# ivclab/CPG

Measured on AMD Instinct MI355X. Metric: images/sec per CPG train-prune-retrain cycle, VGG16 task-1, higher is better.
Workload: dtype f32; 1 GPU; configs[1]: VGG16-BN custom_vgg 224x224, task-1 CPG cycle (finetune -> prune 0.0->0.1 -> recovery, validate after every 20th train step), batch 256 per GPU; task=1, arch=vgg16, global_batch=256, per_gpu_batch=256, parallelism=dp1, epoch_steps=20

## Files before the change

cpg_amd/_lib.py:

```python
import ctypes
import os
import sys

import torch

_HERE = os.path.dirname(os.path.abspath(__file__))
LIB_PATH = os.environ.get('CPG_HIP_LIB') or os.path.join(_HERE, 'lib', 'libcpg_hip.so')

ABI_VERSION = 3
CPG_OK = 0
CPG_E_KRANGE = 2
CPG_E_INVALID = -1
MODE_FINETUNE = 0
MODE_PRUNE = 1



class ConvDesc(ctypes.Structure):
    _fields_ = [(n, ctypes.c_int32) for n in
                ('N', 'C', 'H', 'W', 'K', 'R', 'S', 'stride_h', 'stride_w', 'pad_h', 'pad_w', 'dil_h', 'dil_w', 'groups')]


class PruneResult(ctypes.Structure):
    _fields_ = [('n_candidates', ctypes.c_int64), ('k', ctypes.c_int64), ('n_released', ctypes.c_int64),
# ... 101 lines not shown
    'cpg_conv2d_dgrad_bf16x3': (_int, [_desc, _vp, _vp, _vp, _f32, _vp, _vp, _sz, _vp]),
    'cpg_conv2d_wgrad_bf16x3': (_int, [_desc, _vp, _vp, _vp, _vp, _f32, _vp, _vp, _vp, _sz, _vp]),
    'cpg_conv2d_dgrad_bf16': (_int, [_desc, _vp, _vp, _vp, _f32, _vp, _vp, _sz, _vp]),
    'cpg_conv2d_dgrad_bnbwd_tiles': (_i32, [_desc]),
    'cpg_conv2d_dgrad_bnbwd': (_int, [_desc, _vp, _vp, _vp, _f32, _vp, _vp, _vp, _vp, _vp, _vp, _vp, _sz, _vp, _sz, _vp]),
    'cpg_bn_bwd_from_partials': (_int, [_vp, _i32, _vp, _vp, _vp, _vp, _vp, _vp, _vp, _vp, _vp, _i32, _i32, _i32, _vp, _sz, _vp]),
    'cpg_bn_bwd_finalize_partials': (_int, [_vp, _i32, _i32, _i32, _i32, _vp, _vp, _vp, _vp]),
    'cpg_stem_bn_supported': (_i32, [_desc]),
    'cpg_stem_bn_tiles': (_i32, [_desc]),
    'cpg_stem_bn_stats': (_int, [_desc, _vp, _vp, _vp, _f32, _vp, _vp, _sz, _vp]),
    'cpg_stem_bn_relu_fwd': (_int, [_desc, _vp, _vp, _vp, _f32, _vp, _vp, _vp, _vp, _vp, _vp, _vp]),
    'cpg_stem_bn_relu_bwd_reduce': (_int, [_desc, _vp, _vp, _vp, _f32, _vp, _vp, _vp, _vp, _vp, _vp, _vp, _sz, _vp]),
    'cpg_stem_bn_relu_bwd_apply': (_int, [_desc, _vp, _vp, _vp, _f32, _vp, _vp, _vp, _vp, _vp, _vp, _vp, _vp, _vp]),
    'cpg_stem_bn_wgrad_workspace': (_sz, [_desc]),
    'cpg_stem_bn_relu_bwd_wgrad': (_int, [_desc, _vp, _vp, _vp, _f32, _vp, _vp, _vp, _vp, _vp, _vp, _vp, _vp, _vp, _vp, _sz, _vp]),
    'cpg_bn_stats_finalize_count': (_int, [_vp, _i32, _i32, _i32, _i32, _f32, _f32, _vp, _vp, _vp, _vp, _vp, _vp]),
    'cpg_bn_stats_finalize': (_int, [_vp, _i32, _i32, _i32, _i32, _f32, _f32, _vp, _vp, _vp, _vp, _vp]),
    'cpg_bn_add_relu_mask_bytes': (_sz, [_i32, _i32, _i32]),
    'cpg_bn_add_relu_fwd': (_int, [_vp, _vp, _vp, _vp, _f32, _f32, _vp, _vp, _vp, _vp, _vp, _i32, _i32, _i32, _i32, _vp, _sz, _vp, _vp]),
    'cpg_bn_relu_pool3_supported': (_i32, [_i32, _i32]),
    'cpg_bn_relu_pool3_fwd': (_int, [_vp] * 6 + [_i32] * 4 + [_vp]),
    'cpg_bn_relu_pool3_bwd': (_int, [_vp] * 9 + [_i32] * 5 + [_vp, _sz, _vp]),
    'cpg_bn_add_relu_bwd': (_int, [_vp] * 11 + [_i32] * 4 + [_vp, _sz, _vp, _vp]),
    'cpg_prelu_fwd': (_int, [_vp, _vp, _vp, _vp, _i32, _i32, _i32, _i32, _vp]),
    'cpg_prelu_bwd_bias': (_int, [_vp] * 6 + [_i32] * 4 + [_vp, _sz, _vp]),
    'cpg_prelu_workspace_bytes': (_sz, [_i32, _i32, _i32]),
    'cpg_prelu_bwd': (_int, [_vp, _vp, _vp, _vp, _vp, _i32, _i32, _i32, _i32, _vp, _sz, _vp]),
    'cpg_image_resample_workspace_bytes': (_sz, [ctypes.POINTER(ResampleItem), _i32]),
    'cpg_image_resample': (_int, [_vp, _i64, ctypes.POINTER(ResampleItem), _i32, _vp, _i64, _vp, _sz, _vp]),
    'cpg_image_to_tensor': (_int, [_vp, _i64, ctypes.POINTER(TensorItem), _i32, _i32, _i32, ctypes.POINTER(_f32), ctypes.POINTER(_f32), _vp,
# ... 126 lines not shown
```

cpg_amd/csrc/conv3x3_stem.hip:

```cpp
#include <algorithm>
#include <type_traits>
#include "cpg_dispatch.h"

using namespace cpg;

namespace {

typedef float f32x2 __attribute__((ext_vector_type(2)));
constexpr int ST_R = 8, ST_W = 32;
constexpr int ST_PW = 36;
constexpr int ST_ROWS = ST_R + 2;
constexpr int ST_CMAX = 3, ST_KS = 14;
constexpr int ST_PATCH = ST_CMAX * ST_ROWS * ST_PW;

struct StemGeom {
    int N, C, K, H, W;
    int tiles_x, tiles_y;
    unsigned ntiles;
};

enum { ST_PLAIN = 0, ST_STATS = 1, ST_STATS_ONLY = 2, ST_BN_RELU = 3, ST_BWD_REDUCE = 4, ST_BWD_APPLY = 5, ST_BWD_WGRAD = 6 };
constexpr int ST_TS = 36;
struct StemBn {
    const float *gamma, *beta, *mean, *invstd;
    const float *coef;
    const float *gz;
};

template <int MODE, int NB = 2, bool RAG = false>
__global__ __launch_bounds__(256, 2)
void k_stem_fwd(StemGeom g, const float *__restrict__ x, const float *__restrict__ w, const float *__restrict__ pm, float thr,
                const float *__restrict__ bias, float *__restrict__ y, float *__restrict__ stats, StemBn bn) {
    constexpr bool STATS = MODE == ST_STATS || MODE == ST_STATS_ONLY || MODE == ST_BWD_REDUCE;
    constexpr bool BN = MODE >= ST_BN_RELU;
    constexpr bool STORE = MODE == ST_PLAIN || MODE == ST_STATS || MODE == ST_BN_RELU || MODE == ST_BWD_APPLY;
    constexpr bool WG = MODE == ST_BWD_WGRAD;
    constexpr bool TWO_PASS = STATS || BN;
    __shared__ float smem_all[4 * ST_PATCH];
    __shared__ __attribute__((aligned(16))) float cst[(MODE >= ST_BWD_REDUCE) ? NB * 32 * 8 : 4];
    const int tid = threadIdx.x, lane = tid & 63, wave = __builtin_amdgcn_readfirstlane(tid >> 6);
    if constexpr (MODE >= ST_BWD_REDUCE) {
        if (tid < NB * 32) {
            const bool kv = tid < g.K;
            cst[tid * 8 + 0] = kv ? bn.mean[tid] : 0.0f, cst[tid * 8 + 1] = kv ? bn.invstd[tid] : 0.0f;
            cst[tid * 8 + 2] = kv ? bn.gamma[tid] : 0.0f, cst[tid * 8 + 3] = kv ? bn.beta[tid] : 0.0f;
            cst[tid * 8 + 4] = (MODE >= ST_BWD_APPLY && kv) ? bn.coef[2 * tid] : 0.0f;
            cst[tid * 8 + 5] = (MODE >= ST_BWD_APPLY && kv) ? bn.coef[2 * tid + 1] : 0.0f;
        }
        __syncthreads();
    }
    const int li = lane & 31, lh = lane >> 5;
    float *smem = smem_all + wave * ST_PATCH;
    const int HW = g.H * g.W, CK = g.C * 9;
    __shared__ __attribute__((aligned(16))) float tsm_all[WG ? 4 * 32 * ST_TS : 4];
    float *tsm = tsm_all + (WG ? wave * 32 * ST_TS : 0);
    const int wk = li < CK ? li : 0, wboff = ((wk / 9) * ST_ROWS + (wk % 9) / 3) * ST_PW + wk % 3 + lh;
    f32x16 accw[WG ? NB : 1];
    if constexpr (WG) {
#pragma unroll
        for (int mb = 0; mb < NB; ++mb)
#pragma unroll
            for (int e = 0; e < 16; ++e) accw[mb][e] = 0.0f;
    }

    constexpr bool ALDS = NB == 3 && TWO_PASS;
    __shared__ float a_lds[ALDS ? NB * ST_KS * 64 : 1];
    float A[ALDS ? 1 : NB][ST_KS];
    int boff[ST_KS];
#pragma unroll
    for (int t = 0; t < ST_KS; ++t) {
        const int k = 2 * t + lh;
        const bool kv = k < CK;
#pragma unroll
        for (int mb = 0; mb < NB; ++mb) {
            const int co = mb * 32 + li;
            float v = 0.0f;
            if (kv && co < g.K) {
                v = w[co * CK + k];
                if (pm != nullptr) v *= binarize(pm[co * CK + k], thr);
            }
// ... 46 lines not shown
            const int row = y0 - 1 + r, col = side ? x0 + ST_W : x0 - 1;
            const bool ok = item < ST_CMAX * ST_ROWS && c < g.C && (unsigned)row < (unsigned)g.H && (unsigned)col < (unsigned)g.W;
            const int off = ok ? (((n * g.C + c) * g.H + row) * g.W + col) * 4 : kOOR;
            ph = __builtin_bit_cast(float, __builtin_amdgcn_raw_buffer_load_b32(srd_x, off, 0, 0));
        }
    };
    auto write_patch = [&]() {
#pragma unroll
        for (int q = 0; q < 15; ++q) smem[(2 * q + hw_half) * ST_PW + 1 + hcol] = pc[q];
        if (lane < 2 * ST_CMAX * ST_ROWS) smem[(lane >> 1) * ST_PW + ((lane & 1) ? ST_W + 1 : 0)] = ph;
    };

    if constexpr (ALDS) __syncthreads();
    const unsigned nwaves = gridDim.x * 4, wid = blockIdx.x * 4 + wave;
    if (wid >= g.ntiles) return;
    const int HW4 = HW * 4;
    issue_loads(wid);
    for (unsigned tile = wid; tile < g.ntiles; tile += nwaves) {
        int n, y0, x0;
        tile_coords(tile, n, y0, x0);
        write_patch();
        if (tile + nwaves < g.ntiles) issue_loads(tile + nwaves);
        float s1[16], s2[16];
        auto zero_sums = [&]() {
            if (STATS) {
#pragma unroll
                for (int e = 0; e < 16; ++e) s1[e] = s2[e] = 0.0f;
            }
        };
        const __amdgpu_buffer_rsrc_t srd_y = __builtin_amdgcn_make_buffer_rsrc((void *)((STORE ? y : (float *)x) + (STORE ? (int64_t)n * g.K * HW : 0)), 0, STORE ? g.K * HW4 : 0, 0x00020000);
// ... 82 lines not shown
                    }
                    if constexpr (MODE == ST_STATS || MODE == ST_STATS_ONLY) {
                        const float vm = (FULL || pok) ? v : 0.0f;
                        s1[e] += vm;
                        s2[e] = fmaf(vm, vm, s2[e]);
                    }
                    if constexpr (MODE == ST_BN_RELU) {
                        const float z = relu_keep((v - cm[e]) * cis[e] * cga[e] + cbe[e]);
                        __builtin_amdgcn_raw_buffer_store_b32(__builtin_bit_cast(int, z), srd_y, voff_of(mb, e), cu * HW4, 0);
                    }
                    if constexpr (MODE >= ST_BWD_REDUCE) {
                        const float *cc = cst + (cu + 4 * lh) * 8 + copq;
                        const f32x4 c4 = *reinterpret_cast<const f32x4 *>(cc);
                        const float xh = (v - c4[0]) * c4[1];
                        const float gm = ((v - c4[0]) * c4[1] * c4[2] + c4[3] > 0.0f) ? gzv[e] : 0.0f;
                        if constexpr (MODE == ST_BWD_REDUCE) {
                            s1[e] += gm;
                            s2[e] = fmaf(gm, xh, s2[e]);
                        } else {
                            const f32x2 c2 = *reinterpret_cast<const f32x2 *>(cc + 4);
                            float gyv = (gm - c2[0] - xh * c2[1]) * (c4[1] * c4[2]);
                            if constexpr (MODE == ST_BWD_APPLY) {
                                __builtin_amdgcn_raw_buffer_store_b32(__builtin_bit_cast(int, gyv), srd_y, voff_of(mb, e), cu * HW4, 0);
                            } else {
                                if (!FULL && !pok) gyv = 0.0f;
                                tsm[((e & 3) + 8 * (e >> 2) + 4 * lh) * ST_TS + (li & 1) * 16 + (li >> 1)] = gyv;
                            }
                        }
                    }
                }
            if constexpr (WG) {
                f32x4 ga[4];
#pragma unroll
                for (int q = 0; q < 4; ++q) ga[q] = *reinterpret_cast<const f32x4 *>(tsm + li * ST_TS + lh * 16 + 4 * q);
                const float *brow = smem + j * ST_PW + wboff;
#pragma unroll
                for (int t = 0; t < 16; ++t)
                    accw[MB0] = __builtin_amdgcn_mfma_f32_32x32x2f32(ga[t >> 2][t & 3], brow[2 * t], accw[MB0], 0, 0, 0);
            }
        };
        auto rows = [&](auto mbsel) {
            if (full) {
#pragma unroll 1
                for (int j = 0; j < ST_R; ++j) row(j, std::true_type{}, mbsel);
            } else {
#pragma unroll 1
                for (int j = 0; j < ST_R; ++j) row(j, std::false_type{}, mbsel);
            }
        };
        auto stats_out = [&](int mb) {
#pragma unroll
            for (int e = 0; e < 16; e += 8) half_wave_sum8(s1 + e), half_wave_sum8(s2 + e);
            if (li == kHalfSumLane) {
#pragma unroll
                for (int e = 0; e < 16; ++e) {
                    const int co = mb * 32 + (e & 3) + 8 * (e >> 2) + 4 * lh;
                    if (RAG && co >= g.K) continue;
                    f32x2 o;
                    o[0] = s1[e], o[1] = s2[e];
                    *reinterpret_cast<f32x2 *>(stats + ((int64_t)co * g.ntiles + tile) * 2) = o;
                }
            }
        };
        if (TWO_PASS) {
            load_bn(0);
            zero_sums();
            rows(std::integral_constant<int, 0>{});
            if (STATS) stats_out(0);
            load_bn(1);
            zero_sums();
            rows(std::integral_constant<int, 1>{});
            if (STATS) stats_out(1);
            if constexpr (NB == 3) {
                load_bn(2);
                zero_sums();
                rows(std::integral_constant<int, 2>{});
                if (STATS) stats_out(2);
            }
        } else {
            rows(std::integral_constant<int, -1>{});
        }
    }
    if constexpr (WG) {
        float *dstw = y + (int64_t)wid * g.K * CK;
#pragma unroll
        for (int mb = 0; mb < NB; ++mb)
#pragma unroll
            for (int e = 0; e < 16; ++e) {
                const int co = mb * 32 + (e & 3) + 8 * (e >> 2) + 4 * lh;
                if (li < CK && co < g.K) dstw[co * CK + li] = accw[mb][e];
            }
    }
}

#define STEM_LAUNCH(MODE, grid, block, shm, stream, ...)                                                          \
    do {                                                                                                          \
        if (g.K == 64) hipLaunchKernelGGL((k_stem_fwd<MODE, 2, false>), grid, block, shm, stream, __VA_ARGS__);   \
        else hipLaunchKernelGGL((k_stem_fwd<MODE, 3, true>), grid, block, shm, stream, __VA_ARGS__);              \
    } while (0)

bool stem_geom(int N, int C, int K, int H, int W, StemGeom &g) {
    if (opt_on(OPT_NO_STEM)) return false;
    if (N < 1 || C < 1 || C > ST_CMAX || K < 64 || K > 96 || H < 1 || W < 1) return false;
    if ((int64_t)N * C * H * W * 4 >= (1ll << 31) || (int64_t)K * H * W * 4 >= (1ll << 31)) return false;
    g.N = N, g.C = C, g.K = K, g.H = H, g.W = W;
    g.tiles_x = (W + ST_W - 1) / ST_W, g.tiles_y = (H + ST_R - 1) / ST_R;
// ... 30 lines not shown
}

namespace {
bool stem_bn_geom(const cpg_conv_desc *d, StemGeom &g) {
    if (opt_on(OPT_NO_STEM_FUSE)) return false;
    if (!(d->R == 3 && d->S == 3 && d->stride_h == 1 && d->stride_w == 1 && d->pad_h == 1 && d->pad_w == 1 && d->dil_h == 1 &&
          d->dil_w == 1 && d->groups == 1))
        return false;
    return stem_geom(d->N, d->C, d->K, d->H, d->W, g);
}
unsigned stem_blocks(const StemGeom &g) {
    unsigned blocks = (unsigned)std::min<int64_t>(((int64_t)g.ntiles + 3) / 4, 4 * kCUs);
    blocks = (unsigned)std::max(1, opt_or(OPT_STEM_BLOCKS, (int)blocks));
    return blocks;
}
}

extern "C" int32_t cpg_stem_bn_supported(const cpg_conv_desc *d) {
    StemGeom g;
    return (d != nullptr && stem_bn_geom(d, g)) ? 1 : 0;
}
extern "C" int32_t cpg_stem_bn_tiles(const cpg_conv_desc *d) {
    StemGeom g;
    return (d != nullptr && stem_bn_geom(d, g)) ? (int32_t)g.ntiles : 0;
}
extern "C" int cpg_stem_bn_stats(const cpg_conv_desc *d, const float *x, const float *w, const float *pm, float thr, const float *bias,
                                 float *stats, size_t stats_bytes, void *stream_v) {
    StemGeom g;
    CPG_REQUIRE(d && x && w && stats, "cpg_stem_bn_stats: null pointer");
    if (!stem_bn_geom(d, g)) return fail(CPG_E_UNSUPPORTED, "cpg_stem_bn_stats: shape not supported");
// ... 7 lines not shown
extern "C" int cpg_stem_bn_relu_fwd(const cpg_conv_desc *d, const float *x, const float *w, const float *pm, float thr, const float *bias,
                                    const float *gamma, const float *beta, const float *mean, const float *invstd, float *z, void *stream_v) {
    StemGeom g;
    CPG_REQUIRE(d && x && w && gamma && beta && mean && invstd && z, "cpg_stem_bn_relu_fwd: null pointer");
    if (!stem_bn_geom(d, g)) return fail(CPG_E_UNSUPPORTED, "cpg_stem_bn_relu_fwd: shape not supported");
    if (bias != nullptr) return fail(CPG_E_UNSUPPORTED, "cpg_stem_bn_relu_fwd: the fused stem takes no conv bias");
    STEM_LAUNCH(ST_BN_RELU, dim3(stem_blocks(g)), dim3(256), 0, (hipStream_t)stream_v, g, x, w, pm, thr, bias, z,
                       (float *)nullptr, StemBn{gamma, beta, mean, invstd, nullptr, nullptr});
    CPG_CHECK_LAUNCH("cpg_stem_bn_relu_fwd");
    return CPG_OK;
}
extern "C" int cpg_stem_bn_relu_bwd_reduce(const cpg_conv_desc *d, const float *x, const float *w, const float *pm, float thr,
                                           const float *bias, const float *gamma, const float *beta, const float *mean, const float *invstd,
                                           const float *gz, float *partials, size_t partials_bytes, void *stream_v) {
    StemGeom g;
    CPG_REQUIRE(d && x && w && gamma && beta && mean && invstd && gz && partials, "cpg_stem_bn_relu_bwd_reduce: null pointer");
    if (!stem_bn_geom(d, g)) return fail(CPG_E_UNSUPPORTED, "cpg_stem_bn_relu_bwd_reduce: shape not supported");
    if (bias != nullptr) return fail(CPG_E_UNSUPPORTED, "cpg_stem_bn_relu_bwd_reduce: the fused stem takes no conv bias");
    if (partials_bytes < (size_t)g.K * g.ntiles * 2 * sizeof(float)) return fail(CPG_E_WORKSPACE, "cpg_stem_bn_relu_bwd_reduce: partial-sum buffer too small");
    STEM_LAUNCH(ST_BWD_REDUCE, dim3(stem_blocks(g)), dim3(256), 0, (hipStream_t)stream_v, g, x, w, pm, thr, bias,
                       (float *)nullptr, partials, StemBn{gamma, beta, mean, invstd, nullptr, gz});
    CPG_CHECK_LAUNCH("cpg_stem_bn_relu_bwd_reduce");
    return CPG_OK;
}
extern "C" int cpg_stem_bn_relu_bwd_apply(const cpg_conv_desc *d, const float *x, const float *w, const float *pm, float thr,
                                          const float *bias, const float *gamma, const float *beta, const float *mean, const float *invstd,
                                          const float *coef, const float *gz, float *gy, void *stream_v) {
    StemGeom g;
    CPG_REQUIRE(d && x && w && gamma && beta && mean && invstd && coef && gz && gy, "cpg_stem_bn_relu_bwd_apply: null pointer");
    if (!stem_bn_geom(d, g)) return fail(CPG_E_UNSUPPORTED, "cpg_stem_bn_relu_bwd_apply: shape not supported");
    if (bias != nullptr) return fail(CPG_E_UNSUPPORTED, "cpg_stem_bn_relu_bwd_apply: the fused stem takes no conv bias");
    STEM_LAUNCH(ST_BWD_APPLY, dim3(stem_blocks(g)), dim3(256), 0, (hipStream_t)stream_v, g, x, w, pm, thr, bias, gy,
                       (float *)nullptr, StemBn{gamma, beta, mean, invstd, coef, gz});
    CPG_CHECK_LAUNCH("cpg_stem_bn_relu_bwd_apply");
    return CPG_OK;
}

extern "C" size_t cpg_stem_bn_wgrad_workspace(const cpg_conv_desc *d) {
    StemGeom g;
    if (d == nullptr || !stem_bn_geom(d, g)) return 0;
    return (size_t)stem_blocks(g) * 4 * g.K * g.C * 9 * sizeof(float);
}
extern "C" int cpg_stem_bn_relu_bwd_wgrad(const cpg_conv_desc *d, const float *x, const float *w, const float *pm, float thr,
                                          const float *bias, const float *gamma, const float *beta, const float *mean, const float *invstd,
                                          const float *coef, const float *gz, float *gw, float *gpm, void *ws, size_t ws_bytes,
                                          void *stream_v) {
    StemGeom g;
    CPG_REQUIRE(d && x && w && gamma && beta && mean && invstd && coef && gz && gw && ws, "cpg_stem_bn_relu_bwd_wgrad: null pointer");
    CPG_REQUIRE((pm == nullptr) == (gpm == nullptr), "cpg_stem_bn_relu_bwd_wgrad: piggymask and its gradient come as a pair");
    if (!stem_bn_geom(d, g)) return fail(CPG_E_UNSUPPORTED, "cpg_stem_bn_relu_bwd_wgrad: shape not supported");
    if (bias != nullptr) return fail(CPG_E_UNSUPPORTED, "cpg_stem_bn_relu_bwd_wgrad: the fused stem takes no conv bias");
    const unsigned blocks = stem_blocks(g);
    if (ws_bytes < (size_t)blocks * 4 * g.K * g.C * 9 * sizeof(float)) return fail(CPG_E_WORKSPACE, "cpg_stem_bn_relu_bwd_wgrad: workspace too small");
    hipStream_t stream = (hipStream_t)stream_v;
    STEM_LAUNCH(ST_BWD_WGRAD, dim3(blocks), dim3(256), 0, stream, g, x, w, pm, thr, bias, (float *)ws, (float *)nullptr,
                       StemBn{gamma, beta, mean, invstd, coef, gz});
    const int nsplit = (int)std::min<int64_t>((int64_t)g.ntiles, (int64_t)blocks * 4);
    Epilogue ep{gw, nullptr, BIAS_NONE, 1, 1, pm, w, gpm, thr};
    launch_split_reduce((const float *)ws, nsplit, (int64_t)g.K * g.C * 9, 0, ep, stream);
    CPG_CHECK_LAUNCH("cpg_stem_bn_relu_bwd_wgrad");
    return CPG_OK;
}
```

cpg_amd/csrc/cpg_common.cpp:

```cpp
#include "cpg_common.h"
#include <stdarg.h>
#include <stdlib.h>
#include <string.h>
#include <atomic>

namespace cpg {

static thread_local char g_err[512] = "";

char *err_buf() { return g_err; }

int fail(int code, const char *fmt, ...) {
    va_list ap;
    va_start(ap, fmt);
    vsnprintf(g_err, sizeof(g_err), fmt, ap);
    va_end(ap);
    return code;
}

static thread_local PackCtx g_pack = {};
PackCtx &pack_ctx() { return g_pack; }
static thread_local WgradRider g_rider = {};
WgradRider &wgrad_rider() { return g_rider; }
static thread_local PoolMaxCtx g_pool_max = {};
PoolMaxCtx &pool_max_ctx() { return g_pool_max; }
static thread_local PoolMaxCtx g_bn_pool_max = {};
PoolMaxCtx &bn_pool_max_ctx() { return g_bn_pool_max; }

int take_packed(size_t bytes, const float **pre, const char *what) {
    PackCtx &c = g_pack;
    *pre = nullptr;
    if (!c.armed) return CPG_OK;
    if (c.use == nullptr || c.use_bytes != bytes || (((uintptr_t)c.use) & 15) != 0)
        return fail(CPG_E_INVALID, "%s: the packed operand handed in (%zu bytes) is not the one this launch streams (%zu bytes, 16-byte aligned)",
                    what, c.use_bytes, bytes);
    *pre = c.use;
    c.armed = false;
    return CPG_OK;
}

static std::atomic<int> g_shared_chip{0};
int shared_chip_hint() { return g_shared_chip.load(std::memory_order_relaxed); }
// ... 1 lines not shown
namespace {
enum Kind { BOOL, INT, WINO_KERNEL };
struct OptDef {
    const char *name;
    Kind kind;
};
const OptDef kDefs[OPT_COUNT] = {
    {"CPG_NO_WINO", BOOL},          {"CPG_NO_WINO_WGRAD", BOOL},   {"CPG_NO_WINO_ODD", BOOL},      {"CPG_NO_STEM", BOOL},
    {"CPG_NO_STEM_FUSE", BOOL},     {"CPG_NO_DEAD_SKIP", BOOL},    {"CPG_NO_S2", BOOL},            {"CPG_NO_V14", BOOL},
    {"CPG_DISABLE_CONV3X3", BOOL},  {"CPG_DISABLE_CONV1X1", BOOL}, {"CPG_DISABLE_CONV1X1_WGRAD", BOOL}, {"CPG_DISABLE_PW_GEMM", BOOL},
    {"CPG_C3_FORCE", INT},          {"CPG_C3W_BPC", INT},          {"CPG_W3_PICK", INT},           {"CPG_PWW_BPC", INT},
    {"CPG_STEM_BLOCKS", INT},       {"CPG_WINO_KERNEL", WINO_KERNEL}, {"CPG_WINO_NW", INT},        {"CPG_WINO_PERSIST", INT},
    {"CPG_WINO_GRIDS", INT},        {"CPG_WW_UNITS", INT},         {"CPG_WW_XCD", INT},            {"CPG_PW_TILE", INT},           {"CPG_WG3_SHARE", INT},
    {"CPG_WW_SHARE", INT},          {"CPG_WINO_TAIL", INT},         {"CPG_FC_SMALL", INT},
    {"CPG_NO_WW_RIDER", BOOL},      {"CPG_NO_GROUPED", BOOL},       {"CPG_GROUPED_WIDE_MIN", INT},
    {"CPG_NO_POOL_MAX", BOOL},
};

struct Table {
    std::atomic<int> v[OPT_COUNT];
    Table() {
        for (int i = 0; i < OPT_COUNT; ++i) {
            int val = OPT_UNSET;
            if (const char *f = getenv(kDefs[i].name)) {
                switch (kDefs[i].kind) {
                    case BOOL: val = (f[0] == 0 || (f[0] == '0' && f[1] == 0)) ? 0 : 1; break;
                    case INT: val = atoi(f); break;
                    case WINO_KERNEL: val = f[0] == 'b' ? 0 : f[0] == 'p' ? 2 : f[0] == '6' ? 3 : 1; break;
                }
            }
            v[i].store(val, std::memory_order_relaxed);
// ... 37 lines not shown
```

cpg_amd/csrc/cpg_common.h:

```cpp
#pragma once
#include <hip/hip_runtime.h>
#include <stdint.h>
#include <stdio.h>
#include "../../include/cpg_hip.h"

namespace cpg {

char *err_buf();
int fail(int code, const char *fmt, ...);
int shared_chip_hint();

enum Opt {
    OPT_NO_WINO,
    OPT_NO_WINO_WGRAD,
    OPT_NO_WINO_ODD,
    OPT_NO_STEM,
    OPT_NO_STEM_FUSE,
    OPT_NO_DEAD_SKIP,
    OPT_NO_S2,
    OPT_NO_V14,
    OPT_DISABLE_CONV3X3,
    OPT_DISABLE_CONV1X1,
    OPT_DISABLE_CONV1X1_WGRAD,
    OPT_DISABLE_PW_GEMM,
// ... 5 lines not shown
    OPT_WINO_KERNEL,
    OPT_WINO_NW,
    OPT_WINO_PERSIST,
    OPT_WINO_GRIDS,
    OPT_WW_UNITS,
    OPT_WW_XCD,
    OPT_PW_TILE,
    OPT_WG3_SHARE,
    OPT_WW_SHARE,
    OPT_WINO_TAIL,
    OPT_FC_SMALL,
    OPT_NO_WW_RIDER,
    OPT_NO_GROUPED,
    OPT_GROUPED_WIDE_MIN,
    OPT_NO_POOL_MAX,
    OPT_COUNT
};
constexpr int OPT_UNSET = INT32_MIN;
int opt(Opt o);
inline bool opt_on(Opt o) { const int v = opt(o); return v != OPT_UNSET && v != 0; }
inline int opt_or(Opt o, int dflt) { const int v = opt(o); return v == OPT_UNSET ? dflt : v; }

struct PackJob {
    int family;
    int K, C;
    int a, b, c, d;
    long long total;
    size_t bytes;
};
struct PackCtx {
// ... 9 lines not shown
struct WgradRider {
    bool armed;
    const float *y, *gz, *table;
    float *gy;
    int N, C, HW;
};
WgradRider &wgrad_rider();

struct PoolMaxCtx {
    bool armed;
    float *E;
    size_t bytes;
};
PoolMaxCtx &pool_max_ctx();
PoolMaxCtx &bn_pool_max_ctx();

inline int hip_status(hipError_t e, const char *what) {
    if (e == hipSuccess) return CPG_OK;
    return fail(CPG_E_HIP_BASE + (int)e, "%s: %s", what, hipGetErrorString(e));
}

#define CPG_CHECK_LAUNCH(what)                                   \
    do {                                                         \
        hipError_t e__ = hipGetLastError();                      \
        if (e__ != hipSuccess) return cpg::hip_status(e__, what); \
    } while (0)

#define CPG_REQUIRE(cond, ...)                                  \
    do {                                                        \
        if (!(cond)) return cpg::fail(CPG_E_INVALID, __VA_ARGS__); \
// ... 43 lines not shown
```

cpg_amd/models/fused_bn.py:

```python
import ctypes

import torch
import torch.nn as nn

from .. import _lib
from .layers import BiasGradSink, BnBwdHint, PoolMaxSink, _conv_desc

ENABLED = True
ENABLE_BWD_HINT = False
ENABLE_WGRAD_RIDER = True
RELU_BYTE_MASK = True
FUSE_STEM = True
FUSE_STEM_WGRAD = True
FUSE_SKIP_ADD = True
FUSE_EVAL_BLOCKS = True
FUSE_EVAL_PRELU = False


def _batch_stats(stats, nbt, N, C, HW, eps, momentum, running_mean, running_var, training, device):
    if not training:
        return running_mean, torch.rsqrt(running_var + eps), nbt
    mean = torch.empty(C, dtype=torch.float32, device=device)
    invstd = torch.empty(C, dtype=torch.float32, device=device)
    if stats is not None:
        args = (_lib.dptr(stats, name='bn partial sums'), stats.shape[1], N, C, HW, float(eps), float(momentum),
                _lib.dptr(running_mean, name='running_mean'), _lib.dptr(running_var, name='running_var'), _lib.dptr(mean), _lib.dptr(invstd))
        if nbt is not None and running_mean is not None and nbt.is_cuda and nbt.dtype == torch.int64 and nbt.numel() == 1:
            _lib.call('cpg_bn_stats_finalize_count', *args, _lib.dptr(nbt, torch.int64, 'num_batches_tracked'), _lib.stream_ptr())
# ... 365 lines not shown
        ctx.save_for_backward(x, w, p, gamma, beta, mean, invstd)
        ctx.desc, ctx.thr, ctx.tiles = d, thr, tiles
        return z

    @staticmethod
    def backward(ctx, gz):
        x, w, p, gamma, beta, mean, invstd = ctx.saved_tensors
        d, thr, tiles = ctx.desc, ctx.thr, ctx.tiles
        gz = gz.contiguous()
        L = _lib.lib()
        s = _lib.stream_ptr()
        N, K, H, W = x.shape[0], w.shape[0], x.shape[2], x.shape[3]
        partials = torch.empty((K, tiles, 2), dtype=torch.float32, device=x.device)
        args = (ctypes.byref(d), _lib.dptr(x), _lib.dptr(w), _lib.dptr(p), thr, None, _lib.dptr(gamma), _lib.dptr(beta), _lib.dptr(mean),
                _lib.dptr(invstd))
        _lib.call('cpg_stem_bn_relu_bwd_reduce', *args, _lib.dptr(gz, name='grad_output'), _lib.dptr(partials), partials.numel() * 4, s)
        dgamma, dbeta = torch.empty_like(gamma), torch.empty_like(beta)
        coef = torch.empty(2 * K, dtype=torch.float32, device=x.device)
        _lib.call('cpg_bn_bwd_finalize_partials', _lib.dptr(partials), tiles, N, K, H * W, _lib.dptr(dgamma), _lib.dptr(dbeta), _lib.dptr(coef), s)
        gw = gpm = None
        if ctx.needs_input_grad[1] or (p is not None and ctx.needs_input_grad[2]):
            gw = torch.empty_like(w)
            gpm = None if p is None else torch.empty_like(p)
            if FUSE_STEM_WGRAD:
                ws, nbytes = _lib.workspace(L.cpg_stem_bn_wgrad_workspace(ctypes.byref(d)), x.device)
                _lib.call('cpg_stem_bn_relu_bwd_wgrad', *args, _lib.dptr(coef), _lib.dptr(gz), _lib.dptr(gw), _lib.dptr(gpm), _lib.dptr(ws),
                          nbytes, s)
            else:
                gy = torch.empty((N, K, H, W), dtype=torch.float32, device=x.device)
                _lib.call('cpg_stem_bn_relu_bwd_apply', *args, _lib.dptr(coef), _lib.dptr(gz), _lib.dptr(gy), s)
                ws, nbytes = _lib.workspace(L.cpg_conv2d_workspace_bytes(ctypes.byref(d)), x.device)
                _lib.call('cpg_conv2d_wgrad', ctypes.byref(d), _lib.dptr(x), _lib.dptr(gy), _lib.dptr(w), _lib.dptr(p), thr, _lib.dptr(gw),
                          _lib.dptr(gpm), None, _lib.dptr(ws), nbytes, s)
        return (None, gw, gpm, None, dgamma, dbeta) + (None,) * 5


def stem_conv_bn_relu(conv, bn, x):
    if not (ENABLED and FUSE_STEM and FusedSequential.fuse and hasattr(conv, 'forward_with_bn_stats')
            and _stats_from_conv(bn, FusedSequential.fuse_stats, x, need_grad=True)
            and x.dim() == 4 and x.dtype == torch.float32 and not x.requires_grad
# ... 121 lines not shown
```

include/cpg_hip.h:

```cpp
#ifndef CPG_HIP_H
#define CPG_HIP_H

#include <stddef.h>
#include <stdint.h>

#ifdef __cplusplus
extern "C" {
#endif

#define CPG_ABI_VERSION 3

#define CPG_OK 0
#define CPG_E_INVALID (-1)
#define CPG_E_UNSUPPORTED (-2)
#define CPG_E_WORKSPACE (-3)
#define CPG_E_KRANGE 2
#define CPG_E_HIP_BASE 1000

#define CPG_MODE_FINETUNE 0
#define CPG_MODE_PRUNE 1

typedef struct cpg_conv_desc {
    int32_t N, C, H, W;
    int32_t K;
// ... 183 lines not shown
                      const float *bias, float *stats, size_t stats_bytes, void *stream);
int cpg_stem_bn_relu_fwd(const cpg_conv_desc *desc, const float *x, const float *w, const float *piggymask, float threshold,
                         const float *bias, const float *gamma, const float *beta, const float *mean, const float *invstd, float *z,
                         void *stream);
int cpg_stem_bn_relu_bwd_reduce(const cpg_conv_desc *desc, const float *x, const float *w, const float *piggymask, float threshold,
                                const float *bias, const float *gamma, const float *beta, const float *mean, const float *invstd,
                                const float *gz, float *partials, size_t partials_bytes, void *stream);
int cpg_stem_bn_relu_bwd_apply(const cpg_conv_desc *desc, const float *x, const float *w, const float *piggymask, float threshold,
                               const float *bias, const float *gamma, const float *beta, const float *mean, const float *invstd,
                               const float *coef, const float *gz, float *gy, void *stream);
size_t cpg_stem_bn_wgrad_workspace(const cpg_conv_desc *desc);
int cpg_stem_bn_relu_bwd_wgrad(const cpg_conv_desc *desc, const float *x, const float *w, const float *piggymask, float threshold,
                               const float *bias, const float *gamma, const float *beta, const float *mean, const float *invstd,
                               const float *coef, const float *gz, float *gw, float *gpm, void *workspace, size_t workspace_bytes,
                               void *stream);

size_t cpg_bn_add_relu_mask_bytes(int32_t N, int32_t C, int32_t HW);
int cpg_bn_add_relu_fwd(const float *x, const float *res, const float *gamma, const float *beta, float eps,
                        float momentum, float *running_mean, float *running_var, float *mean, float *invstd, float *y,
                        int32_t N, int32_t C, int32_t HW, int32_t train, void *ws, size_t ws_bytes, void *stream, uint8_t *relu_mask);
int cpg_bn_add_relu_bwd(const float *x, const float *out, const float *gy, const float *gamma, const float *beta,
                        const float *mean, const float *invstd, float *gx, float *gz, float *dgamma, float *dbeta, int32_t N,
                        int32_t C, int32_t HW, int32_t train, void *ws, size_t ws_bytes, void *stream, const uint8_t *relu_mask);

int cpg_bn_relu_pool_fwd(const float *x, const float *gamma, const float *beta, float eps, float momentum,
                         float *running_mean, float *running_var, float *mean, float *invstd, float *y_pooled,
                         int32_t N, int32_t C, int32_t H, int32_t W, int32_t train, void *ws, size_t ws_bytes,
                         void *stream);
int cpg_bn_relu_pool_bwd(const float *x, const float *g_pooled, const float *gamma, const float *beta,
                         const float *mean, const float *invstd, float *gx, float *dgamma, float *dbeta,
// ... 69 lines not shown
```

Baseline: 2438 images/sec.

## Fuse stem BN backward reduce and weight-gradient into a single pass

Adds a one-pass backward for the fused stem conv+BN+ReLU. The BN-stat reduction kernel now also accumulates the masked-gradient weight products and an input Gram matrix via MFMA. A small finish kernel then algebraically applies the BN coefficient correction in double precision, so the separate second pass over the input and grad_output is no longer needed. It is armed through a thread-local context keyed on the workspace pointer. The extra MFMA work, LDS stores and Gram matrix raise per-tile cost, and the cancellation-style correction may lose accuracy.

Measured after the change: 2456 images/sec (median of 6 runs). No clear change (+0.7%).

```diff
diff --git a/cpg_amd/_lib.py b/cpg_amd/_lib.py
--- a/cpg_amd/_lib.py
+++ b/cpg_amd/_lib.py
@@ -139,6 +139,9 @@
     'cpg_stem_bn_relu_bwd_apply': (_int, [_desc, _vp, _vp, _vp, _f32, _vp, _vp, _vp, _vp, _vp, _vp, _vp, _vp, _vp]),
     'cpg_stem_bn_wgrad_workspace': (_sz, [_desc]),
     'cpg_stem_bn_relu_bwd_wgrad': (_int, [_desc, _vp, _vp, _vp, _f32, _vp, _vp, _vp, _vp, _vp, _vp, _vp, _vp, _vp, _vp, _sz, _vp]),
+    'cpg_stem_bn_onepass_supported': (_i32, [_desc]),
+    'cpg_stem_bn_onepass_workspace': (_sz, [_desc]),
+    'cpg_stem_bn_relu_bwd_attach_onepass': (_int, [_vp, _sz]),
     'cpg_bn_stats_finalize_count': (_int, [_vp, _i32, _i32, _i32, _i32, _f32, _f32, _vp, _vp, _vp, _vp, _vp, _vp]),
     'cpg_bn_stats_finalize': (_int, [_vp, _i32, _i32, _i32, _i32, _f32, _f32, _vp, _vp, _vp, _vp, _vp]),
     'cpg_bn_add_relu_mask_bytes': (_sz, [_i32, _i32, _i32]),
diff --git a/cpg_amd/csrc/conv3x3_stem.hip b/cpg_amd/csrc/conv3x3_stem.hip
--- a/cpg_amd/csrc/conv3x3_stem.hip
+++ b/cpg_amd/csrc/conv3x3_stem.hip
@@ -19,7 +19,7 @@
     unsigned ntiles;
 };
 
-enum { ST_PLAIN = 0, ST_STATS = 1, ST_STATS_ONLY = 2, ST_BN_RELU = 3, ST_BWD_REDUCE = 4, ST_BWD_APPLY = 5, ST_BWD_WGRAD = 6 };
+enum { ST_PLAIN = 0, ST_STATS = 1, ST_STATS_ONLY = 2, ST_BN_RELU = 3, ST_BWD_REDUCE = 4, ST_BWD_APPLY = 5, ST_BWD_WGRAD = 6, ST_BWD_ONEPASS = 7 };
 constexpr int ST_TS = 36;
 struct StemBn {
     const float *gamma, *beta, *mean, *invstd;
@@ -31,10 +31,12 @@
 __global__ __launch_bounds__(256, 2)
 void k_stem_fwd(StemGeom g, const float *__restrict__ x, const float *__restrict__ w, const float *__restrict__ pm, float thr,
                 const float *__restrict__ bias, float *__restrict__ y, float *__restrict__ stats, StemBn bn) {
-    constexpr bool STATS = MODE == ST_STATS || MODE == ST_STATS_ONLY || MODE == ST_BWD_REDUCE;
+    constexpr bool ONEPASS = MODE == ST_BWD_ONEPASS;
+    constexpr bool STATS = MODE == ST_STATS || MODE == ST_STATS_ONLY || MODE == ST_BWD_REDUCE || ONEPASS;
     constexpr bool BN = MODE >= ST_BN_RELU;
     constexpr bool STORE = MODE == ST_PLAIN || MODE == ST_STATS || MODE == ST_BN_RELU || MODE == ST_BWD_APPLY;
-    constexpr bool WG = MODE == ST_BWD_WGRAD;
+    constexpr bool WG = MODE == ST_BWD_WGRAD || ONEPASS;
+    constexpr bool COEF = MODE == ST_BWD_APPLY || MODE == ST_BWD_WGRAD;
     constexpr bool TWO_PASS = STATS || BN;
     __shared__ float smem_all[4 * ST_PATCH];
     __shared__ __attribute__((aligned(16))) float cst[(MODE >= ST_BWD_REDUCE) ? NB * 32 * 8 : 4];
@@ -44,8 +46,8 @@
             const bool kv = tid < g.K;
             cst[tid * 8 + 0] = kv ? bn.mean[tid] : 0.0f, cst[tid * 8 + 1] = kv ? bn.invstd[tid] : 0.0f;
             cst[tid * 8 + 2] = kv ? bn.gamma[tid] : 0.0f, cst[tid * 8 + 3] = kv ? bn.beta[tid] : 0.0f;
-            cst[tid * 8 + 4] = (MODE >= ST_BWD_APPLY && kv) ? bn.coef[2 * tid] : 0.0f;
-            cst[tid * 8 + 5] = (MODE >= ST_BWD_APPLY && kv) ? bn.coef[2 * tid + 1] : 0.0f;
+            cst[tid * 8 + 4] = (COEF && kv) ? bn.coef[2 * tid] : 0.0f;
+            cst[tid * 8 + 5] = (COEF && kv) ? bn.coef[2 * tid + 1] : 0.0f;
         }
         __syncthreads();
     }
@@ -56,14 +58,17 @@
     float *tsm = tsm_all + (WG ? wave * 32 * ST_TS : 0);
     const int wk = li < CK ? li : 0, wboff = ((wk / 9) * ST_ROWS + (wk % 9) / 3) * ST_PW + wk % 3 + lh;
     f32x16 accw[WG ? NB : 1];
+    f32x16 accq;
     if constexpr (WG) {
 #pragma unroll
         for (int mb = 0; mb < NB; ++mb)
 #pragma unroll
             for (int e = 0; e < 16; ++e) accw[mb][e] = 0.0f;
-    }
-
-    constexpr bool ALDS = NB == 3 && TWO_PASS;
+#pragma unroll
+        for (int e = 0; e < 16; ++e) accq[e] = 0.0f;
+    }
+
+    constexpr bool ALDS = (NB == 3 && TWO_PASS) || ONEPASS;
     __shared__ float a_lds[ALDS ? NB * ST_KS * 64 : 1];
     float A[ALDS ? 1 : NB][ST_KS];
     int boff[ST_KS];
@@ -140,6 +145,7 @@
     if constexpr (ALDS) __syncthreads();
     const unsigned nwaves = gridDim.x * 4, wid = blockIdx.x * 4 + wave;
     if (wid >= g.ntiles) return;
+    if constexpr (ONEPASS) __builtin_assume(wid < g.ntiles);
     const int HW4 = HW * 4;
     issue_loads(wid);
     for (unsigned tile = wid; tile < g.ntiles; tile += nwaves) {
@@ -252,9 +258,10 @@
                         const f32x4 c4 = *reinterpret_cast<const f32x4 *>(cc);
                         const float xh = (v - c4[0]) * c4[1];
                         const float gm = ((v - c4[0]) * c4[1] * c4[2] + c4[3] > 0.0f) ? gzv[e] : 0.0f;
-                        if constexpr (MODE == ST_BWD_REDUCE) {
+                        if constexpr (MODE == ST_BWD_REDUCE || ONEPASS) {
                             s1[e] += gm;
                             s2[e] = fmaf(gm, xh, s2[e]);
+                            if constexpr (ONEPASS) tsm[((e & 3) + 8 * (e >> 2) + 4 * lh) * ST_TS + (li & 1) * 16 + (li >> 1)] = gm;
                         } else {
                             const f32x2 c2 = *reinterpret_cast<const f32x2 *>(cc + 4);
                             float gyv = (gm - c2[0] - xh * c2[1]) * (c4[1] * c4[2]);
@@ -273,8 +280,15 @@
                 for (int q = 0; q < 4; ++q) ga[q] = *reinterpret_cast<const f32x4 *>(tsm + li * ST_TS + lh * 16 + 4 * q);
                 const float *brow = smem + j * ST_PW + wboff;
 #pragma unroll
-                for (int t = 0; t < 16; ++t)
-                    accw[MB0] = __builtin_amdgcn_mfma_f32_32x32x2f32(ga[t >> 2][t & 3], brow[2 * t], accw[MB0], 0, 0, 0);
+                for (int t = 0; t < 16; ++t) {
+                    float b = brow[2 * t];
+                    if constexpr (ONEPASS) b = li == CK ? 1.0f : b;
+                    accw[MB0] = __builtin_amdgcn_mfma_f32_32x32x2f32(ga[t >> 2][t & 3], b, accw[MB0], 0, 0, 0);
+                    if constexpr (ONEPASS && MB0 == 0) {
+                        const float a = (FULL || (y0 + j < g.H && x0 + 2 * t + lh < g.W)) ? b : 0.0f;
+                        accq = __builtin_amdgcn_mfma_f32_32x32x2f32(a, b, accq, 0, 0, 0);
+                    }
+                }
             }
         };
         auto rows = [&](auto mbsel) {
@@ -289,6 +303,8 @@
         auto stats_out = [&](int mb) {
 #pragma unroll
             for (int e = 0; e < 16; e += 8) half_wave_sum8(s1 + e), half_wave_sum8(s2 + e);
+            unsigned nt = g.ntiles;
+            if constexpr (ONEPASS) asm volatile("" : "+s"(nt));
             if (li == kHalfSumLane) {
 #pragma unroll
                 for (int e = 0; e < 16; ++e) {
@@ -296,7 +312,8 @@
                     if (RAG && co >= g.K) continue;
                     f32x2 o;
                     o[0] = s1[e], o[1] = s2[e];
-                    *reinterpret_cast<f32x2 *>(stats + ((int64_t)co * g.ntiles + tile) * 2) = o;
+                    if constexpr (ONEPASS) *reinterpret_cast<f32x2 *>(stats + ((int64_t)co * nt + tile) * 2) = o;
+                    else *reinterpret_cast<f32x2 *>(stats + ((int64_t)co * g.ntiles + tile) * 2) = o;
                 }
             }
         };
@@ -320,14 +337,28 @@
         }
     }
     if constexpr (WG) {
-        float *dstw = y + (int64_t)wid * g.K * CK;
-#pragma unroll
-        for (int mb = 0; mb < NB; ++mb)
-#pragma unroll
-            for (int e = 0; e < 16; ++e) {
-                const int co = mb * 32 + (e & 3) + 8 * (e >> 2) + 4 * lh;
-                if (li < CK && co < g.K) dstw[co * CK + li] = accw[mb][e];
-            }
+        if constexpr (ONEPASS) {
+            unsigned wq = wid;
+            int lq = 4 * lh;
+            asm volatile("" : "+s"(wq), "+v"(lq));
+            float *dstw = y + (int64_t)wq * (g.K * CK + 32 * 32);
+#pragma unroll
+            for (int mb = 0; mb < NB; ++mb)
+#pragma unroll
+                for (int e = 0; e < 16; ++e)
+                    if (li < CK) dstw[(mb * 32 + (e & 3) + 8 * (e >> 2) + lq) * CK + li] = accw[mb][e];
+#pragma unroll
+            for (int e = 0; e < 16; ++e) dstw[g.K * CK + ((e & 3) + 8 * (e >> 2) + lq) * 32 + li] = accq[e];
+        } else {
+            float *dstw = y + (int64_t)wid * g.K * CK;
+#pragma unroll
+            for (int mb = 0; mb < NB; ++mb)
+#pragma unroll
+                for (int e = 0; e < 16; ++e) {
+                    const int co = mb * 32 + (e & 3) + 8 * (e >> 2) + 4 * lh;
+                    if (li < CK && co < g.K) dstw[co * CK + li] = accw[mb][e];
+                }
+        }
     }
 }
 
@@ -388,6 +419,49 @@
     blocks = (unsigned)std::max(1, opt_or(OPT_STEM_BLOCKS, (int)blocks));
     return blocks;
 }
+
+bool onepass_ok(const StemGeom &g) { return g.K == 64 && !opt_on(OPT_NO_STEM_ONEPASS); }
+int onepass_elems(const StemGeom &g) { return g.K * g.C * 9 + 32 * 32; }
+size_t onepass_bytes(const StemGeom &g) {
+    return (size_t)stem_blocks(g) * 4 * onepass_elems(g) * sizeof(float) + 8 + (size_t)onepass_elems(g) * sizeof(double);
+}
+double *onepass_sums(void *ws, const StemGeom &g) {
+    const uintptr_t p = (uintptr_t)ws + (size_t)stem_blocks(g) * 4 * onepass_elems(g) * sizeof(float);
+    return (double *)((p + 7) & ~(uintptr_t)7);
+}
+
+__global__ __launch_bounds__(256) void k_stem_onepass_sum(const float *__restrict__ part, int nsplit, int E, int ks, double *__restrict__ sums) {
+    __shared__ double red[256];
+    const int tid = threadIdx.x, P = 256 / ks, pl = tid % P, sl = tid / P;
+    const int p = blockIdx.x * P + pl;
+    double s = 0.0;
+    if (p < E)
+        for (int k = sl; k < nsplit; k += ks) s += (double)part[(int64_t)k * E + p];
+    red[tid] = s;
+    __syncthreads();
+    if (sl == 0 && p < E) {
+        for (int j = 1; j < ks; ++j) s += red[j * P + pl];
+        sums[p] = s;
+    }
+}
+
+__global__ __launch_bounds__(256) void k_stem_onepass_finish(const double *__restrict__ sums, int K, int CK, const float *__restrict__ w,
+                                                           const float *__restrict__ pm, float thr, StemBn bn, Epilogue ep) {
+    const int i = blockIdx.x * 256 + threadIdx.x;
+    if (i >= K * CK) return;
+    const int k = i / CK, t = i % CK;
+    const double *Q = sums + K * CK;
+    double wq = 0.0;
+    for (int tp = 0; tp < CK; ++tp) {
+        float wv = w[k * CK + tp];
+        if (pm != nullptr) wv *= binarize(pm[k * CK + tp], thr);
+        wq += (double)wv * Q[tp * 32 + t];
+    }
+    const double P = Q[CK * 32 + t], is = (double)bn.invstd[k];
+    const double X = is * (wq - (double)bn.mean[k] * P);
+    const double gv = (double)bn.gamma[k] * is * (sums[i] - (double)bn.coef[2 * k] * P - (double)bn.coef[2 * k + 1] * X);
+    epilogue_store(ep, i, (float)gv);
+}
 }
 
 extern "C" int32_t cpg_stem_bn_supported(const cpg_conv_desc *d) {
@@ -425,10 +499,22 @@
                                            const float *bias, const float *gamma, const float *beta, const float *mean, const float *invstd,
                                            const float *gz, float *partials, size_t partials_bytes, void *stream_v) {
     StemGeom g;
+    StemOnepassCtx &op = stem_onepass_ctx();
+    const bool onepass = op.stage == StemOnepassCtx::ARMED;
+    op.stage = StemOnepassCtx::IDLE;
     CPG_REQUIRE(d && x && w && gamma && beta && mean && invstd && gz && partials, "cpg_stem_bn_relu_bwd_reduce: null pointer");
     if (!stem_bn_geom(d, g)) return fail(CPG_E_UNSUPPORTED, "cpg_stem_bn_relu_bwd_reduce: shape not supported");
     if (bias != nullptr) return fail(CPG_E_UNSUPPORTED, "cpg_stem_bn_relu_bwd_reduce: the fused stem takes no conv bias");
     if (partials_bytes < (size_t)g.K * g.ntiles * 2 * sizeof(float)) return fail(CPG_E_WORKSPACE, "cpg_stem_bn_relu_bwd_reduce: partial-sum buffer too small");
+    if (onepass) {
+        if (!onepass_ok(g)) return fail(CPG_E_UNSUPPORTED, "cpg_stem_bn_relu_bwd_reduce: no one-pass backward for this shape");
+        if (op.bytes < onepass_bytes(g)) return fail(CPG_E_WORKSPACE, "cpg_stem_bn_relu_bwd_reduce: the attached workspace is too small");
+        hipLaunchKernelGGL((k_stem_fwd<ST_BWD_ONEPASS, 2, false>), dim3(stem_blocks(g)), dim3(256), 0, (hipStream_t)stream_v, g, x, w, pm, thr,
+                           bias, (float *)op.ws, partials, StemBn{gamma, beta, mean, invstd, nullptr, gz});
+        CPG_CHECK_LAUNCH("cpg_stem_bn_relu_bwd_reduce");
+        op.stage = StemOnepassCtx::FILLED, op.gz = gz, op.x = x;
+        return CPG_OK;
+    }
     STEM_LAUNCH(ST_BWD_REDUCE, dim3(stem_blocks(g)), dim3(256), 0, (hipStream_t)stream_v, g, x, w, pm, thr, bias,
                        (float *)nullptr, partials, StemBn{gamma, beta, mean, invstd, nullptr, gz});
     CPG_CHECK_LAUNCH("cpg_stem_bn_relu_bwd_reduce");
@@ -457,18 +543,53 @@
                                           const float *coef, const float *gz, float *gw, float *gpm, void *ws, size_t ws_bytes,
                                           void *stream_v) {
     StemGeom g;
+    StemOnepassCtx &op = stem_onepass_ctx();
+    const bool filled = op.stage == StemOnepassCtx::FILLED && op.ws == ws && op.gz == gz && op.x == x;
+    op.stage = StemOnepassCtx::IDLE;
     CPG_REQUIRE(d && x && w && gamma && beta && mean && invstd && coef && gz && gw && ws, "cpg_stem_bn_relu_bwd_wgrad: null pointer");
     CPG_REQUIRE((pm == nullptr) == (gpm == nullptr), "cpg_stem_bn_relu_bwd_wgrad: piggymask and its gradient come as a pair");
     if (!stem_bn_geom(d, g)) return fail(CPG_E_UNSUPPORTED, "cpg_stem_bn_relu_bwd_wgrad: shape not supported");
     if (bias != nullptr) return fail(CPG_E_UNSUPPORTED, "cpg_stem_bn_relu_bwd_wgrad: the fused stem takes no conv bias");
     const unsigned blocks = stem_blocks(g);
+    hipStream_t stream = (hipStream_t)stream_v;
+    const int nsplit = (int)std::min<int64_t>((int64_t)g.ntiles, (int64_t)blocks * 4);
+    Epilogue ep{gw, nullptr, BIAS_NONE, 1, 1, pm, w, gpm, thr};
+    if (filled) {
+        if (!onepass_ok(g)) return fail(CPG_E_UNSUPPORTED, "cpg_stem_bn_relu_bwd_wgrad: no one-pass backward for this shape");
+        if (ws_bytes < onepass_bytes(g)) return fail(CPG_E_WORKSPACE, "cpg_stem_bn_relu_bwd_wgrad: workspace too small");
+        const int E = onepass_elems(g);
+        int ks = 1;
+        while (ks < 64 && ks * 2 <= nsplit && E * ks < 262144) ks *= 2;
+        double *sums = onepass_sums(ws, g);
+        hipLaunchKernelGGL(k_stem_onepass_sum, dim3((unsigned)((E + 256 / ks - 1) / (256 / ks))), dim3(256), 0, stream, (const float *)ws, nsplit, E,
+                           ks, sums);
+        hipLaunchKernelGGL(k_stem_onepass_finish, dim3((unsigned)((g.K * g.C * 9 + 255) / 256)), dim3(256), 0, stream, (const double *)sums, g.K,
+                           g.C * 9, w, pm, thr, StemBn{gamma, beta, mean, invstd, coef, gz}, ep);
+        CPG_CHECK_LAUNCH("cpg_stem_bn_relu_bwd_wgrad");
+        return CPG_OK;
+    }
     if (ws_bytes < (size_t)blocks * 4 * g.K * g.C * 9 * sizeof(float)) return fail(CPG_E_WORKSPACE, "cpg_stem_bn_relu_bwd_wgrad: workspace too small");
-    hipStream_t stream = (hipStream_t)stream_v;
     STEM_LAUNCH(ST_BWD_WGRAD, dim3(blocks), dim3(256), 0, stream, g, x, w, pm, thr, bias, (float *)ws, (float *)nullptr,
                        StemBn{gamma, beta, mean, invstd, coef, gz});
-    const int nsplit = (int)std::min<int64_t>((int64_t)g.ntiles, (int64_t)blocks * 4);
-    Epilogue ep{gw, nullptr, BIAS_NONE, 1, 1, pm, w, gpm, thr};
     launch_split_reduce((const float *)ws, nsplit, (int64_t)g.K * g.C * 9, 0, ep, stream);
     CPG_CHECK_LAUNCH("cpg_stem_bn_relu_bwd_wgrad");
     return CPG_OK;
 }
+
+extern "C" int32_t cpg_stem_bn_onepass_supported(const cpg_conv_desc *d) {
+    StemGeom g;
+    return (d != nullptr && stem_bn_geom(d, g) && onepass_ok(g)) ? 1 : 0;
+}
+extern "C" size_t cpg_stem_bn_onepass_workspace(const cpg_conv_desc *d) {
+    StemGeom g;
+    if (d == nullptr || !stem_bn_geom(d, g) || !onepass_ok(g)) return 0;
+    return onepass_bytes(g);
+}
+extern "C" int cpg_stem_bn_relu_bwd_attach_onepass(void *ws, size_t ws_bytes) {
+    StemOnepassCtx &op = stem_onepass_ctx();
+    op.stage = StemOnepassCtx::IDLE;
+    if (ws == nullptr && ws_bytes == 0) return CPG_OK;
+    CPG_REQUIRE(ws != nullptr && (((uintptr_t)ws) & 3) == 0 && ws_bytes > 0, "cpg_stem_bn_relu_bwd_attach_onepass: needs a 4-byte aligned, non-empty workspace");
+    op.stage = StemOnepassCtx::ARMED, op.ws = ws, op.bytes = ws_bytes, op.gz = op.x = nullptr;
+    return CPG_OK;
+}
diff --git a/cpg_amd/csrc/cpg_common.cpp b/cpg_amd/csrc/cpg_common.cpp
--- a/cpg_amd/csrc/cpg_common.cpp
+++ b/cpg_amd/csrc/cpg_common.cpp
@@ -26,6 +26,8 @@
 PoolMaxCtx &pool_max_ctx() { return g_pool_max; }
 static thread_local PoolMaxCtx g_bn_pool_max = {};
 PoolMaxCtx &bn_pool_max_ctx() { return g_bn_pool_max; }
+static thread_local StemOnepassCtx g_stem_onepass = {};
+StemOnepassCtx &stem_onepass_ctx() { return g_stem_onepass; }
 
 int take_packed(size_t bytes, const float **pre, const char *what) {
     PackCtx &c = g_pack;
@@ -57,7 +59,7 @@
     {"CPG_WINO_GRIDS", INT},        {"CPG_WW_UNITS", INT},         {"CPG_WW_XCD", INT},            {"CPG_PW_TILE", INT},           {"CPG_WG3_SHARE", INT},
     {"CPG_WW_SHARE", INT},          {"CPG_WINO_TAIL", INT},         {"CPG_FC_SMALL", INT},
     {"CPG_NO_WW_RIDER", BOOL},      {"CPG_NO_GROUPED", BOOL},       {"CPG_GROUPED_WIDE_MIN", INT},
-    {"CPG_NO_POOL_MAX", BOOL},
+    {"CPG_NO_POOL_MAX", BOOL},      {"CPG_NO_STEM_ONEPASS", BOOL},
 };
 
 struct Table {
diff --git a/cpg_amd/csrc/cpg_common.h b/cpg_amd/csrc/cpg_common.h
--- a/cpg_amd/csrc/cpg_common.h
+++ b/cpg_amd/csrc/cpg_common.h
@@ -43,6 +43,7 @@
     OPT_NO_GROUPED,
     OPT_GROUPED_WIDE_MIN,
     OPT_NO_POOL_MAX,
+    OPT_NO_STEM_ONEPASS,
     OPT_COUNT
 };
 constexpr int OPT_UNSET = INT32_MIN;
@@ -82,6 +83,15 @@
 };
 PoolMaxCtx &pool_max_ctx();
 PoolMaxCtx &bn_pool_max_ctx();
+
+struct StemOnepassCtx {
+    enum { IDLE = 0, ARMED = 1, FILLED = 2 };
+    int stage;
+    void *ws;
+    size_t bytes;
+    const float *gz, *x;
+};
+StemOnepassCtx &stem_onepass_ctx();
 
 inline int hip_status(hipError_t e, const char *what) {
     if (e == hipSuccess) return CPG_OK;
diff --git a/cpg_amd/models/fused_bn.py b/cpg_amd/models/fused_bn.py
--- a/cpg_amd/models/fused_bn.py
+++ b/cpg_amd/models/fused_bn.py
@@ -12,6 +12,7 @@
 RELU_BYTE_MASK = True
 FUSE_STEM = True
 FUSE_STEM_WGRAD = True
+FUSE_STEM_ONEPASS = True
 FUSE_SKIP_ADD = True
 FUSE_EVAL_BLOCKS = True
 FUSE_EVAL_PRELU = False
@@ -407,16 +408,22 @@
         partials = torch.empty((K, tiles, 2), dtype=torch.float32, device=x.device)
         args = (ctypes.byref(d), _lib.dptr(x), _lib.dptr(w), _lib.dptr(p), thr, None, _lib.dptr(gamma), _lib.dptr(beta), _lib.dptr(mean),
                 _lib.dptr(invstd))
+        want_gw = ctx.needs_input_grad[1] or (p is not None and ctx.needs_input_grad[2])
+        ws = None
+        if want_gw and FUSE_STEM_WGRAD and FUSE_STEM_ONEPASS and L.cpg_stem_bn_onepass_supported(ctypes.byref(d)):
+            ws, nbytes = _lib.workspace(L.cpg_stem_bn_onepass_workspace(ctypes.byref(d)), x.device)
+            _lib.call('cpg_stem_bn_relu_bwd_attach_onepass', _lib.dptr(ws), nbytes)
         _lib.call('cpg_stem_bn_relu_bwd_reduce', *args, _lib.dptr(gz, name='grad_output'), _lib.dptr(partials), partials.numel() * 4, s)
         dgamma, dbeta = torch.empty_like(gamma), torch.empty_like(beta)
         coef = torch.empty(2 * K, dtype=torch.float32, device=x.device)
         _lib.call('cpg_bn_bwd_finalize_partials', _lib.dptr(partials), tiles, N, K, H * W, _lib.dptr(dgamma), _lib.dptr(dbeta), _lib.dptr(coef), s)
         gw = gpm = None
-        if ctx.needs_input_grad[1] or (p is not None and ctx.needs_input_grad[2]):
+        if want_gw:
             gw = torch.empty_like(w)
             gpm = None if p is None else torch.empty_like(p)
             if FUSE_STEM_WGRAD:
-                ws, nbytes = _lib.workspace(L.cpg_stem_bn_wgrad_workspace(ctypes.byref(d)), x.device)
+                if ws is None:
+                    ws, nbytes = _lib.workspace(L.cpg_stem_bn_wgrad_workspace(ctypes.byref(d)), x.device)
                 _lib.call('cpg_stem_bn_relu_bwd_wgrad', *args, _lib.dptr(coef), _lib.dptr(gz), _lib.dptr(gw), _lib.dptr(gpm), _lib.dptr(ws),
                           nbytes, s)
             else:
diff --git a/include/cpg_hip.h b/include/cpg_hip.h
--- a/include/cpg_hip.h
+++ b/include/cpg_hip.h
@@ -221,6 +221,9 @@
                                const float *bias, const float *gamma, const float *beta, const float *mean, const float *invstd,
                                const float *coef, const float *gz, float *gw, float *gpm, void *workspace, size_t workspace_bytes,
                                void *stream);
+int32_t cpg_stem_bn_onepass_supported(const cpg_conv_desc *desc);
+size_t cpg_stem_bn_onepass_workspace(const cpg_conv_desc *desc);
+int cpg_stem_bn_relu_bwd_attach_onepass(void *workspace, size_t workspace_bytes);
 
 size_t cpg_bn_add_relu_mask_bytes(int32_t N, int32_t C, int32_t HW);
 int cpg_bn_add_relu_fwd(const float *x, const float *res, const float *gamma, const float *beta, float eps,
```
